# david-cortes/cmfrec

Hardware: AMD Instinct MI355X
Metric: ALS rows/sec ((users+items)/iteration time), implicit ALS-CG k=50 fp64 (higher is better)
Workload: dtype f64

## Files before the change

cmfrec_amd/_lib.py:

```python
import ctypes as C
import os

import numpy as np

_HERE = os.path.dirname(os.path.abspath(__file__))
LIBDIR = os.environ.get("CMFREC_HIP_LIBDIR") or os.path.join(_HERE, "lib")

RETURN_CODES = {0: "ok", 1: "out of memory", 2: "invalid or unsupported input", 3: "interrupted",
                4: "HIP runtime failure"}


class Model(C.Structure):
    _fields_ = [(n, C.c_int32) for n in (
        "implicit", "m", "n", "k", "k_main", "k_user", "k_item", "user_bias", "item_bias",
        "scale_lam", "scale_lam_sideinfo", "use_cg", "precondition_cg", "max_cg_steps",
        "p", "q", "m_u", "n_i")] + [("lam", C.c_double), ("w_user", C.c_double), ("w_item", C.c_double)] + \
        [(n, C.c_int32) for n in ("row_begin", "row_end", "col_begin", "col_end", "m_x", "n_x")]


class ModelF(C.Structure):
    _fields_ = [(n, C.c_int32) for n in (
        "implicit", "m", "n", "k", "k_main", "k_user", "k_item", "user_bias", "item_bias",
        "scale_lam", "scale_lam_sideinfo", "use_cg", "precondition_cg", "max_cg_steps",
        "p", "q", "m_u", "n_i")] + [("lam", C.c_float), ("w_user", C.c_float), ("w_item", C.c_float)] + \
        [(n, C.c_int32) for n in ("row_begin", "row_end", "col_begin", "col_end", "m_x", "n_x")]


EXPORTED = [
    "fit_collective_implicit_als", "fit_collective_explicit_als",
    "factors_collective_explicit_multiple", "factors_collective_implicit_multiple", "cmfrec_hip_factors_multiple", "cmfrec_hip_factors_multiple_l1",
    "cmfrec_hip_optimizeA_implicit", "cmfrec_hip_optimizeA_explicit", "cmfrec_hip_optimizeA_explicit_weighted",
    "cmfrec_hip_optimizeA_dense_full", "cmfrec_hip_optimizeA_collective", "cmfrec_hip_optimizeA_collective_sparse", "cmfrec_hip_topN_batch",
    "cmfrec_hip_ranker_create", "cmfrec_hip_ranker_topN", "cmfrec_hip_ranker_kernel_ms", "cmfrec_hip_ranker_launch_shape", "cmfrec_hip_ranker_destroy",
    "cmfrec_hip_session_create", "cmfrec_hip_session_destroy", "cmfrec_hip_last_error", "cmfrec_hip_last_error_code",
    "cmfrec_hip_session_set_X", "cmfrec_hip_session_set_A_parts", "cmfrec_hip_session_nparts", "cmfrec_hip_session_part_range", "cmfrec_hip_session_stream_wait_part", "cmfrec_hip_session_set_X_coo", "cmfrec_hip_session_set_X_coo_weighted", "cmfrec_hip_session_set_X_weighted", "cmfrec_hip_session_set_X_coo_device", "cmfrec_hip_session_precompute", "cmfrec_hip_session_init_biases", "cmfrec_hip_session_get_X", "cmfrec_hip_session_set_factors", "cmfrec_hip_session_get_factors",
    "cmfrec_hip_session_set_sideinfo", "cmfrec_hip_session_set_sideinfo_local", "cmfrec_hip_session_sideinfo_partial", "cmfrec_hip_session_sideinfo_finish", "cmfrec_hip_session_set_nonneg", "cmfrec_hip_session_set_l1", "cmfrec_hip_session_set_lam_unique", "cmfrec_hip_session_set_scale_bias_const", "cmfrec_hip_session_set_NA_as_zero_X", "cmfrec_hip_session_set_zero_rows", "cmfrec_hip_session_set_closed_form_rows", "cmfrec_hip_session_set_lambda_multipliers", "cmfrec_hip_session_set_implicit_features", "cmfrec_hip_session_get_implicit_features", "cmfrec_hip_session_set_sideinfo_sparse", "cmfrec_hip_session_update", "cmfrec_hip_session_iterate",
    "cmfrec_hip_session_sync", "cmfrec_hip_session_device_ptr", "cmfrec_hip_session_stream",
    "cmfrec_hip_session_after_gather", "cmfrec_hip_session_kernel_time",
    "cmfrec_hip_session_reset_timers", "cmfrec_hip_session_bin_overlaps", "cmfrec_hip_session_vh_mode", "cmfrec_hip_session_vh_min", "cmfrec_hip_session_lowrank_info", "cmfrec_hip_session_bin_stats", "cmfrec_hip_sizeof_real", "cmfrec_hip_sizeof_model", "cmfrec_hip_build_info", "cmfrec_hip_reload_switches", "cmfrec_hip_selftest_lanes", "cmfrec_hip_exchange_plan", "cmfrec_hip_gemm_probe", "cmfrec_hip_sym_eig", "precompute_collective_explicit", "precompute_collective_implicit", "topN_old_collective_explicit", "topN_old_collective_implicit", "cmfrec_hip_random_parallel",
]

_cache = {}


def lib_path(dtype):
    suffix = "double" if np.dtype(dtype) == np.float64 else "float"
    return os.path.join(LIBDIR, "libcmfrec_hip_%s.so" % suffix)


def load(dtype=np.float64):
    dtype = np.dtype(dtype).type
    if dtype not in (np.float64, np.float32):
        raise ValueError("dtype must be float64 or float32")
    if dtype in _cache:
        return _cache[dtype]
    path = lib_path(dtype)
    if not os.path.exists(path):
        raise ImportError(
            "%s is missing: the HIP extension has not been built (run __graft_entry__.build() or "
            "`make -C cmfrec_amd/csrc`). cmfrec_amd has no CPU fallback." % path)
    if os.environ.get("CMFREC_AMD_NO_TORCH_PRELOAD") != "1":
        try:
            import torch
        except ImportError:
            pass
    lib = C.CDLL(path)
    lib.cmfrec_hip_last_error.restype = C.c_char_p
    lib.cmfrec_hip_build_info.restype = C.c_char_p
    lib.cmfrec_hip_session_create.restype = C.c_void_p
    lib.cmfrec_hip_ranker_create.restype = C.c_void_p
    lib.cmfrec_hip_ranker_destroy.restype = None
    lib.cmfrec_hip_session_device_ptr.restype = C.c_void_p
    lib.cmfrec_hip_session_stream.restype = C.c_void_p
    assert lib.cmfrec_hip_sizeof_real() == np.dtype(dtype).itemsize
    mirror = Model if dtype is np.float64 else ModelF
    if lib.cmfrec_hip_sizeof_model() != C.sizeof(mirror):
        raise RuntimeError("cmfrec_amd: the ctypes mirror of cmfrec_hip_model (%d bytes) does not match the library (%d)"
                           % (C.sizeof(mirror), lib.cmfrec_hip_sizeof_model()))
    _cache[dtype] = lib
    return lib


def real(dtype):
    return C.c_double if np.dtype(dtype) == np.float64 else C.c_float


def ptr(a):
    return None if a is None else a.ctypes.data_as(C.c_void_p)


def check(rc, lib, what, interrupt_ok=False):
    if rc == 0 or (rc == 3 and interrupt_ok):
        return
    msg = lib.cmfrec_hip_last_error()
    msg = msg.decode() if msg else ""
    if rc == 1:
        raise MemoryError("%s: out of memory. %s" % (what, msg))
    if rc == 3:
        raise InterruptedError("%s: procedure was interrupted" % what)
    raise RuntimeError("%s failed with code %d (%s). %s" % (what, rc, RETURN_CODES.get(rc, "?"), msg))
```

cmfrec_amd/csrc/cg_kernels.hpp:

```cpp
#pragma once
#include <hip/hip_runtime.h>
#include <stdint.h>
#include <type_traits>

#include "lanes.hpp"

namespace cmfhip {

constexpr int WAVE = 64;
constexpr int TILE = 64;
constexpr int MAX_W = 8;
#ifndef CMF_CG_WAVES_PER_SIMD
#define CMF_CG_WAVES_PER_SIMD 2
#endif
#ifndef CMF_CG_WAVES_PER_SIMD_F32
#define CMF_CG_WAVES_PER_SIMD_F32 3
#endif
#ifndef CMF_CG_WAVES_PER_SIMD_LOW
#define CMF_CG_WAVES_PER_SIMD_LOW 3
#endif
constexpr int CG_NTSEL_MAX_S = 7;
template <typename T, int W, int NRES_, int NTSEL = 0> constexpr int cg_waves_per_simd()
{
    if (sizeof(T) == 8 && NTSEL == 1 && W <= 8) return CMF_CG_WAVES_PER_SIMD_LOW;
// ... 931 lines not shown
        for (int q = 0; q < 4; q++) {
            const f32x2 *g = reinterpret_cast<const f32x2 *>(G) + (jj * 4 + q) * gram_ld2(S) + ll;
#pragma unroll
            for (int s = 0; s < S; s++) v[q][s] = g[8 * s];
        }
    }
};
template <int S>
__device__ __forceinline__ void gram_pass_regs(const GramRegs<float, S> &R, float wdist, PassAcc<float> &out)
{
    float wts[8];
    wts[0] = lanes::bcast8<0>(wdist); wts[1] = lanes::bcast8<1>(wdist); wts[2] = lanes::bcast8<2>(wdist);
    wts[3] = lanes::bcast8<3>(wdist); wts[4] = lanes::bcast8<4>(wdist); wts[5] = lanes::bcast8<5>(wdist);
    wts[6] = lanes::bcast8<6>(wdist); wts[7] = lanes::bcast8<7>(wdist);
#pragma unroll
    for (int q = 0; q < 4; q++) {
        const f32x2 w2 = f32x2{wts[2 * q], wts[2 * q + 1]};
#pragma unroll
        for (int s = 0; s < S; s++) out.v[s] += w2 * R.v[q][s];
    }
}
template <typename T, int S>
__device__ __forceinline__ void gram_pass_regs(const GramRegs<T, S> &R, T wdist, PassAcc<T> &out)
{
    T wts[8];
    wts[0] = lanes::bcast8<0>(wdist); wts[1] = lanes::bcast8<1>(wdist); wts[2] = lanes::bcast8<2>(wdist);
    wts[3] = lanes::bcast8<3>(wdist); wts[4] = lanes::bcast8<4>(wdist); wts[5] = lanes::bcast8<5>(wdist);
    wts[6] = lanes::bcast8<6>(wdist); wts[7] = lanes::bcast8<7>(wdist);
#pragma unroll
    for (int t = 0; t < 8; t++)
#pragma unroll
        for (int s = 0; s < S; s++) out.v[s] += wts[t] * R.v[t][s];
}

template <bool NEG, int S>
__device__ __forceinline__ void gram_pass_regs_w(const GramRegs<float, S> &R, const float (&wts)[8], PassAcc<float> &out)
{
#pragma unroll
    for (int q = 0; q < 4; q++) {
        const f32x2 w2 = f32x2{wts[2 * q], wts[2 * q + 1]};
#pragma unroll
        for (int s = 0; s < S; s++) out.v[s] = NEG ? out.v[s] - w2 * R.v[q][s] : out.v[s] + w2 * R.v[q][s];
    }
}
template <bool NEG, typename T, int S, int GR>
__device__ __forceinline__ void gram_pass_regs_w(const GramRegs<T, S, GR> &R, const T (&wts)[8], PassAcc<T> &out)
{
#pragma unroll
    for (int t = 0; t < GR; t++)
#pragma unroll
        for (int s = 0; s < S; s++) out.v[s] = NEG ? out.v[s] - wts[t] * R.v[t][s] : out.v[s] + wts[t] * R.v[t][s];
}

template <typename T, int S, bool IMPLICIT, bool GRAMX = false, int NE = 4>
__global__ void __launch_bounds__(256, (tiny_waves_per_simd<T, IMPLICIT || GRAMX>()))
cg_rows_tiny_kernel(const CgParams<T> P)
{
    static_assert(NE == 4 || NE == 2 || NE == 0, "entries per lane group");
    constexpr bool MIX = NE == 0;
    static_assert(!MIX || CMF_TINY_WAVES_PER_SIMD >= 3, "the mixed launch lives in the dynamically scheduled loop");
    using Tile = typename TinyTile<T, S, (NE == 2) ? 2 : 4>::type;
    constexpr bool GRAM = IMPLICIT || GRAMX;
    extern __shared__ __attribute__((aligned(16))) unsigned char smem_raw[];
    T *G = reinterpret_cast<T *>(smem_raw);
    constexpr bool PV = pass_vector_in_lds<T>();
    __shared__ __attribute__((aligned(16))) T s_pv[PV ? 4 : 1][PV ? 64 : 1];
    const int tid = threadIdx.x;
    const int lane = tid & 63;
    auto short_row = [&](int nnz_) -> bool { return MIX && nnz_ <= 16; };
    auto entry_of = [&](int nnz_) -> int { return (NE == 2 || short_row(nnz_)) ? (lane >> 2) : (lane >> 1); };
    const int k = P.k;
    constexpr bool GREG = tiny_greg<T, GRAM>();
    constexpr int GR = GREG ? gram_rows<T>(S) : 8;
    if (GRAM) {
        stage_gramian<T, S, GR>(G, P.BtB, k, tid, blockDim.x);
        __syncthreads();
    }
    GramRegs<T, GREG ? S : 1, GREG ? GR : 8> greg;
    if constexpr (GREG) greg.load(G, lane);
    const int nwaves = gridDim.x * 4;
    struct Pre { int idx; T x; T a; T g; };
    auto load_desc = [&](int rix_) -> RowDesc {
        RowDesc d; d.row = 0; d.nnz = 0; d.st = 0;
        if (rix_ < P.nrows) d = P.desc[rix_];
        d.row = __builtin_amdgcn_readfirstlane(d.row);
        d.nnz = __builtin_amdgcn_readfirstlane(d.nnz);
        d.st = ((unsigned long long)(unsigned)__builtin_amdgcn_readfirstlane((int)(d.st >> 32)) << 32) |
               (unsigned)__builtin_amdgcn_readfirstlane((int)(d.st & 0xffffffffu));
        return d;
    };
    auto load_pre = [&](const RowDesc &d) -> Pre {
        Pre q; q.idx = 0; q.x = T(0); q.a = T(0); q.g = T(1);
        const int ent = entry_of(d.nnz);
        if (ent < d.nnz) {
            const size_t pos = d.st + (size_t)ent;
            q.idx = P.indices[pos];
            q.x = P.values[pos];
            q.g = entry_weight<T, IMPLICIT>(P, pos);
            if (!IMPLICIT && P.bias_sub != nullptr) q.x -= P.bias_sub[q.idx];
        }
        if (d.nnz > 0 && lane < k) q.a = P.A[(size_t)d.row * P.lda + lane];
        return q;
    };
    auto load_tile_ne = [&](Tile &t_, const T *Bm_, size_t ldb_, int k_, int idx_, int cnt_, int lane_) {
        if constexpr (NE != 2) load_tile4<T, S>(t_, Bm_, ldb_, k_, idx_, cnt_, lane_);
        else load_tile2<T, S>(t_, Bm_, ldb_, k_, idx_, cnt_, lane_);
    };
    auto solve = [&](const RowDesc &d, const Pre &pr, const Tile &tile, auto short_tag) {
        constexpr bool T2 = NE == 2 || decltype(short_tag)::value;
        const int nnz = d.nnz;
        T lam = P.lam, lam_last = P.lam_last;
        if (GRAMX && P.kc > 0) {
            if (P.scale_lam || P.scale_lam_sideinfo) {
                T mult = row_lam_mult(P, d.row, nnz);
                if (P.scale_lam_sideinfo) mult += (T)P.p_side;
                lam *= mult; lam_last *= mult;
            }
        } else if (!IMPLICIT && P.scale_lam) {
            const T mult = row_lam_mult(P, d.row, nnz);
            lam *= mult;
            if (!P.scale_bias_const) lam_last *= mult;
        }
        const bool valid = (T2 ? (lane >> 2) : (lane >> 1)) < nnz;
        T a_d = pr.a;
        auto run_pass = [&](T vdist, auto mode_tag) -> T {
            constexpr int MODE = decltype(mode_tag)::value;
            asm volatile("" ::: "memory");
            T vrep[S];
            T gw[8];
            if constexpr (PV) pass_vector_lds<T, S, GR>(vdist, vrep, gw, lane, &s_pv[tid >> 6][0]);
            else replicate<T, S>(vdist, vrep, lane);
            PassAcc<T> acc;
            if (!CMF_DBG(P, 4)) {
                if constexpr (!T2) tile_pass4<T, S, IMPLICIT, MODE, decltype(tile), true>(tile, vrep, pr.x, valid, acc, lane, pr.g);
                else tile_pass2<T, S, IMPLICIT, MODE, decltype(tile), true>(tile, vrep, pr.x, valid, acc, lane, pr.g);
            } else acc.zero();
            if constexpr (GREG) {
                if (!CMF_DBG(P, 2)) {
                    if constexpr (PV) gram_pass_regs_w<MODE == 0>(greg, gw, acc);
                    else gram_pass_regs(greg, (MODE == 0) ? -vdist : vdist, acc);
                }
            }
            else if (GRAM && !CMF_DBG(P, 2)) gram_pass<T, S, 1>(G, (MODE == 0) ? -vdist : vdist, acc, lane, 0);
            T out[8];
            acc.close(out);
            return treduce8_high<T>(out, lane);
        };
        T r_d = run_pass(a_d, std::integral_constant<int, 0>{});
        r_d -= lam * a_d;
        if (!IMPLICIT && lam != lam_last && lane == k - 1) r_d -= (lam_last - lam) * a_d;
        if (GRAMX && P.rconst != nullptr && lane < k) r_d += P.rconst[(size_t)d.row * P.ldr + lane];
        if (lane >= k) r_d = T(0);
        T p_d = r_d;
        T r_old = wave_sum(r_d * r_d);
        bool done = (r_old <= (T)1e-12);
        for (int step = 0; step < P.max_cg_steps && !done; step++) {
            T Ap_d = run_pass(p_d, std::integral_constant<int, 1>{});
            Ap_d += lam * p_d;
            if (!IMPLICIT && lam != lam_last && lane == k - 1) Ap_d += (lam_last - lam) * p_d;
            if (lane >= k) Ap_d = T(0);
            T alpha = cg_div(r_old, wave_sum(Ap_d * p_d));
            a_d += alpha * p_d;
            r_d -= alpha * Ap_d;
            T r_new = wave_sum(r_d * r_d);
            if (r_new <= (T)1e-8) done = true;
            else {
                p_d = p_d * cg_div(r_new, r_old) + r_d;
                r_old = r_new;
            }
        }
        if (lane < k) P.A[(size_t)d.row * P.lda + lane] = a_d;
    };

    int rix = blockIdx.x * 4 + (tid >> 6);
#if CMF_TINY_WAVES_PER_SIMD >= 3
    {
        const int cslot = rix % CG_NCOUNTERS;
        int *const my_counter = P.counter + cslot * CG_COUNTER_STRIDE;
        const int cbase = nwaves + cslot;
        auto issue_claim = [&]() -> int {
            int v = 0;
            if (lane == 0) v = atomicAdd(my_counter, 1);
            return v;
        };
        const int c1 = issue_claim(), c2 = issue_claim();
        int rnxt = cbase + CG_NCOUNTERS * __builtin_amdgcn_readfirstlane(c1);
        int rnn = cbase + CG_NCOUNTERS * __builtin_amdgcn_readfirstlane(c2);
        RowDesc d0 = load_desc(rix), d1 = load_desc(rnxt);
        Pre p0 = load_pre(d0);
        Tile tA;
        int pend = issue_claim();
        while (rix < P.nrows) {
            const bool shrt = short_row(d0.nnz);
            if (CMF_DBG(P, 1)) {
                dbg_fill_tile<(NE == 2) ? 2 : 4, S>(tA, (T)(p0.idx & 3) * (T)0.001);
            } else if constexpr (MIX) {
                if (shrt) load_tile2<T, S>(tA, P.B, P.ldb, k, p0.idx, d0.nnz, lane);
                else load_tile_ne(tA, P.B, P.ldb, k, p0.idx, d0.nnz, lane);
            } else load_tile_ne(tA, P.B, P.ldb, k, p0.idx, d0.nnz, lane);
            RowDesc d2 = load_desc(rnn);
            Pre p1 = load_pre(d1);
            if constexpr (MIX) {
                if (shrt) solve(d0, p0, tA, std::true_type{});
                else solve(d0, p0, tA, std::false_type{});
            } else solve(d0, p0, tA, std::false_type{});
            const int r3 = cbase + CG_NCOUNTERS * __builtin_amdgcn_readfirstlane(pend);
            d0 = d1; p0 = p1; d1 = d2;
            rix = rnxt; rnxt = rnn; rnn = r3;
            pend = issue_claim();
        }
        return;
    }
#endif
    RowDesc d0 = load_desc(rix), d1 = load_desc(rix + nwaves), d2 = load_desc(rix + 2 * nwaves);
    Pre p0 = load_pre(d0);
    Tile tA, tB;
    if (d0.nnz > 0) load_tile_ne(tA, P.B, P.ldb, k, p0.idx, d0.nnz, lane);
    Pre p1 = load_pre(d1);
    while (rix < P.nrows) {
        if (d1.nnz > 0) load_tile_ne(tB, P.B, P.ldb, k, p1.idx, d1.nnz, lane);
        RowDesc d3 = load_desc(rix + 3 * nwaves);
        Pre p2 = load_pre(d2);
        solve(d0, p0, tA, std::false_type{});
        rix += nwaves;
        if (rix >= P.nrows) break;
        if (d2.nnz > 0) load_tile_ne(tA, P.B, P.ldb, k, p2.idx, d2.nnz, lane);
        RowDesc d4 = load_desc(rix + 3 * nwaves);
        Pre p3 = load_pre(d3);
        solve(d1, p1, tB, std::false_type{});
        rix += nwaves;
        d0 = d2; p0 = p2; d1 = d3; p1 = p3; d2 = d4;
    }
}

constexpr int VH_CHUNK_TILES = 4;

struct VhWork {
    int vi;
    int row;
    int cnt;
    int chunk;
    unsigned long long st;
    unsigned long long pad_;
};

template <typename T>
struct VhState {
    T *r, *p;
    T *r_old;
    int *done;
    T *part;
    const int *chunk_row;
    const int *chunk_start;
    const int *chunk_cnt;
    const int *chunk_off;
    const int *launch;
    const VhWork *work;
    int nvh, nchunks, nlaunch;
};

template <typename T, int S, bool IMPLICIT, int MODE>
__global__ void __launch_bounds__(64 * VH_CHUNK_TILES, 3)
vh_pass_kernel(const CgParams<T> P, const VhState<T> V)
// ... 439 lines not shown
```

cmfrec_amd/csrc/device.hpp:

```cpp
#pragma once
#include <hip/hip_runtime.h>
#include <algorithm>
#include <cstdio>
#include <cstdlib>
#include <cstring>
#include <numeric>
#include <string>
#include <vector>

#include "../../include/cmfrec_hip.h"
#include "device_base.hpp"
#include "cg_kernels.hpp"
#include "chol_kernels.hpp"
#include "dense_kernels.hpp"
#include "gram_cg_kernels.hpp"
#include "topn_kernels.hpp"

namespace cmfhip {

constexpr int MAX_DEVICES = 16;
constexpr int NBINS = 6;
constexpr int BIN_VHEAVY = 0;
constexpr int BIN_HEAVY = 1;
constexpr int BIN_MED4 = 2;
constexpr int BIN_MED2 = 3;
constexpr int BIN_LIGHT = 4;
constexpr int BIN_TINY = 5;
constexpr int BIN_MIN_NNZ[NBINS] = {1025, 257, 129, 65, 33, 1};
inline int vh_min_env()
{
    const int v = switches().vh_min;
    return v > 0 ? std::min(sizeof(real_t) == 4 ? BIN_MIN_NNZ[BIN_VHEAVY] : (1 << 30), std::max(258, v)) : 0;
}

struct SparseShard {
    int nrows = 0;
    size_t nnz = 0;
    int vh_min = BIN_MIN_NNZ[BIN_VHEAVY];
    size_t opp_row_bytes_hint = 50 * sizeof(real_t);
    int bin_of(long long l) const
    {
        if (l >= vh_min) return BIN_VHEAVY;
        for (int b = 1; b < NBINS; b++)
            if (l >= BIN_MIN_NNZ[b]) return b;
        return -1;
    }
    static bool gram_pays(double vh_nnz, int n_other_, size_t opp_bytes_per_row)
    {
        (void)vh_nnz; (void)opp_bytes_per_row;
        return sizeof(real_t) == 4 || n_other_ > 0;
    }
    DevBuf<size_t> p;
    DevBuf<int> i;
    DevBuf<real_t> v;
    DevBuf<real_t> w, wsum;
// ... 354 lines not shown
    volatile unsigned int *w = poison_words;
    for (int e = threadIdx.x; e < words; e += 256) w[e] = 0xFFFFFFFFu;
}
inline void poison_lds(hipStream_t st, int num_cus)
{
    if (!switches().poison_lds) return;
    constexpr int BYTES = 80 * 1024;
    static thread_local bool attr_set = false;
    if (!attr_set) {
        HIP_CHECK(hipFuncSetAttribute((const void *)poison_lds_kernel, hipFuncAttributeMaxDynamicSharedMemorySize, BYTES));
        attr_set = true;
    }
    hipLaunchKernelGGL(poison_lds_kernel, dim3(num_cus * 4), dim3(256), BYTES, st, BYTES / 4);
    HIP_CHECK(hipGetLastError());
}

template <int S, bool IMPLICIT, int W, int RPB, bool GRAMX = false, int NRES_ = 0, int NTSEL = 0>
inline void launch_cg_bin(const DeviceInfo &dev, CgParams<real_t> P, int first, int count, BinTimers *tm, int bin, hipStream_t st, int counter_set = -1)
{
    if (count <= 0) return;
    EventPair ev{nullptr, nullptr};
    if (tm) {
        HIP_CHECK(hipEventCreate(&ev.a));
        HIP_CHECK(hipEventCreate(&ev.b));
        HIP_CHECK(hipEventRecord(ev.a, st));
    }
    poison_lds(st, dev.num_cus);
    P.order += first;
    P.desc += first;
    P.nrows = count;
    P.counter = dev.row_counter.ptr + cg_counter_offset(counter_set >= 0 ? counter_set : bin);
    constexpr int threads = 64 * W * RPB;
    size_t smem = (((IMPLICIT || GRAMX) ? (size_t)gram_elems<real_t>(S) : 0) + (size_t)RPB * 2 * W * 64) * sizeof(real_t);
    auto kern = cg_rows_kernel<real_t, S, IMPLICIT, W, RPB, GRAMX, NRES_, NTSEL>;
    static thread_local int bpc_dev[MAX_DEVICES] = {0};
    int &blocks_per_cu = bpc_dev[std::min(std::max(dev.device, 0), MAX_DEVICES - 1)];
    if (blocks_per_cu == 0) {
        if (smem > 48 * 1024)
            HIP_CHECK(hipFuncSetAttribute((const void *)kern, hipFuncAttributeMaxDynamicSharedMemorySize, (int)smem));
        int nb = 0;
        HIP_CHECK(hipOccupancyMaxActiveBlocksPerMultiprocessor(&nb, kern, threads, smem));
        blocks_per_cu = std::max(1, nb);
    }
    int teams_needed = (count + RPB - 1) / RPB;
    int grid = std::min(teams_needed, dev.num_cus * blocks_per_cu);
    hipLaunchKernelGGL(kern, dim3(grid), dim3(threads), smem, st, P);
    HIP_CHECK(hipGetLastError());
    if (tm) {
        HIP_CHECK(hipEventRecord(ev.b, st));
        tm->ev[bin].push_back(ev);
    }
}

template <int S, bool IMPLICIT, bool GRAMX = false>
inline void launch_cg_tiny(const DeviceInfo &dev, CgParams<real_t> P, int first, int count, BinTimers *tm, hipStream_t st, int n_gt16)
{
    if (count <= 0) return;
    EventPair ev{nullptr, nullptr};
    if (tm) {
        HIP_CHECK(hipEventCreate(&ev.a));
        HIP_CHECK(hipEventCreate(&ev.b));
        HIP_CHECK(hipEventRecord(ev.a, st));
    }
    poison_lds(st, dev.num_cus);
    constexpr bool tiny16_on = true;
    const int count_le16 = std::min(count, std::max(0, first + count - std::max(first, n_gt16)));
    size_t smem = ((IMPLICIT || GRAMX) ? (size_t)gram_elems<real_t>(S) : 0) * sizeof(real_t);
    const int di = std::min(std::max(dev.device, 0), MAX_DEVICES - 1);
    CgParams<real_t> P1 = P;
    P1.order += first;
    P1.desc += first;
    P1.nrows = count;
    P1.counter = dev.row_counter.ptr + cg_counter_offset(BIN_TINY);
    {
        const bool mixed = tiny16_on && count_le16 > 0;
        auto kern = mixed ? cg_rows_tiny_kernel<real_t, S, IMPLICIT, GRAMX, 0> : cg_rows_tiny_kernel<real_t, S, IMPLICIT, GRAMX, 4>;
        static thread_local int bpc_dev[MAX_DEVICES][2] = {{0}};
        int &blocks_per_cu = bpc_dev[di][mixed ? 1 : 0];
        if (blocks_per_cu == 0) {
            int nb = 0;
            HIP_CHECK(hipOccupancyMaxActiveBlocksPerMultiprocessor(&nb, kern, 256, smem));
            blocks_per_cu = std::max(1, nb);
        }
        const int grid = std::min((count + 3) / 4, dev.num_cus * blocks_per_cu);
        hipLaunchKernelGGL(kern, dim3(grid), dim3(256), smem, st, P1);
    }
    HIP_CHECK(hipGetLastError());
    if (tm) {
        HIP_CHECK(hipEventRecord(ev.b, st));
        tm->ev[BIN_TINY].push_back(ev);
    }
}

void launch_gram_wave(dim3 grid, hipStream_t st, const CgParams<real_t> &P, const GramParams<real_t> &G, bool implicit, int rem);

template <bool GRAMX>
inline bool vh_takes_gram(int k, const SparseShard &X)
{
    if (GRAMX || k > 16 * GRAM_NTT) return false;
    return (switches().vh != 0) ? switches().vh == 2 : X.prefer_gram((size_t)k * sizeof(real_t));
}

template <int S, bool IMPLICIT, bool GRAMX = false>
inline void launch_cg_vheavy(const DeviceInfo &dev_, CgParams<real_t> P, const SparseShard &X, BinTimers *tm, hipStream_t st)
{
    const int nvh = X.bin_rows[BIN_VHEAVY];
    if (nvh <= 0) return;
    struct { hipStream_t stream; int num_cus; } dev{st, dev_.num_cus};
    EventPair ev{nullptr, nullptr};
    if (tm) {
        HIP_CHECK(hipEventCreate(&ev.a));
        HIP_CHECK(hipEventCreate(&ev.b));
        HIP_CHECK(hipEventRecord(ev.a, dev.stream));
    }
    if (vh_takes_gram<GRAMX>(P.k, X)) {
        GramParams<real_t> G;
        G.sl_vrow = X.sl_vrow.ptr; G.sl_first = X.sl_first.ptr; G.sl_count = X.sl_count.ptr; G.row_sl_off = X.row_sl_off.ptr;
        G.part = X.gram_part.ptr; G.n_slices = X.n_slices; G.nvh = nvh;
        P.nrows = nvh;
#ifdef CMF_CG_DEBUG
        if (switches().debug_ticks) {
            static unsigned long long *d_t = nullptr;
            unsigned long long h[4];
            if (d_t == nullptr) { HIP_CHECK(hipMalloc((void **)&d_t, sizeof(h))); HIP_CHECK(hipMemset(d_t, 0, sizeof(h))); }
            else {
                HIP_CHECK(hipDeviceSynchronize());
                HIP_CHECK(hipMemcpy(h, d_t, sizeof(h), hipMemcpyDeviceToHost));
                if (h[1] > 0)
                    fprintf(stderr, "gram_wave: %.0f ticks per wave, %llu waves, %llu slices, %llu nnz: %.1f ticks per nnz and wave\n",
                            (double)h[0] / h[1], h[1], h[2], h[3], (double)h[0] / (double)h[3]);
                HIP_CHECK(hipMemset(d_t, 0, sizeof(h)));
            }
// ... 328 lines not shown
```

cmfrec_amd/csrc/device_base.hpp:

```cpp
#pragma once
#include <hip/hip_runtime.h>
#include <cstdio>
#include <cstdlib>
#include <cstring>
#include <functional>
#include <new>
#include <string>

#include "../../include/cmfrec_hip.h"

namespace cmfhip {

extern thread_local std::string g_last_error;
extern thread_local int g_last_rc;

struct HipError {
    int code;
};

inline void hip_check(hipError_t e, const char *what, const char *file, int line)
{
    if (e == hipSuccess) return;
    char buf[512];
    snprintf(buf, sizeof buf, "cmfrec_hip: %s failed: %s (%s:%d)", what, hipGetErrorString(e), file, line);
    g_last_error = buf;
    fprintf(stderr, "%s\n", buf);
    throw HipError{e == hipErrorOutOfMemory ? 1 : 4};
}
#define HIP_CHECK(x) ::cmfhip::hip_check((x), #x, __FILE__, __LINE__)

inline int guarded(const std::function<int()> &f)
{
    try {
        return f();
    } catch (const HipError &e) {
        return e.code;
    } catch (const std::bad_alloc &) {
        g_last_error = "cmfrec_hip: host out of memory";
        return 1;
    }
}

struct Switches {
    bool poison_lds = false;
    int vh_min = 0;
    int vh = 0;
    bool gram_slice = false;
    int bins_par = 2;
    bool nt_split = true;
    bool cg_generic = false;
    int chol = 0;
    int parts_coop = 1;
    int chol_wg = 2;
    int gramk = -1;
    int gramk_batch = 0;
    int lowrank = -1;
    bool topn_wide = false;
    int topn_tiles = 0;
    bool eig_jacobi = false;
    int debug_skip = 0;
    bool debug_ticks = false;
    void reload()
    {
        auto str = [](const char *n) -> const char * { const char *v = getenv(n); return (v != nullptr && v[0] != 0) ? v : nullptr; };
        auto num = [&](const char *n, int dflt) -> int { const char *v = str(n); return v ? atoi(v) : dflt; };
        poison_lds = str("CMFREC_HIP_POISON_LDS") != nullptr;
        vh_min = num("CMFREC_HIP_VH_MIN", 0);
        const char *v = str("CMFREC_HIP_VH");
        vh = !v ? 0 : strcmp(v, "stream") == 0 ? 1 : strcmp(v, "gram") == 0 ? 2 : 1;
        v = str("CMFREC_HIP_GRAM_KERNEL"); gram_slice = v && strcmp(v, "slice") == 0;
        bins_par = num("CMFREC_HIP_BINS_PAR", 2);
        nt_split = num("CMFREC_HIP_NT_SPLIT", 1) != 0;
        v = str("CMFREC_HIP_CG_KERNEL"); cg_generic = v && strcmp(v, "generic") == 0;
        v = str("CMFREC_HIP_CHOL"); chol = !v ? 0 : strcmp(v, "rows") == 0 ? 1 : strcmp(v, "noslices") == 0 ? 2 : 0;
        parts_coop = num("CMFREC_HIP_PARTS_COOP", 1);
        chol_wg = num("CMFREC_HIP_CHOL_WG", 2);
        if (chol_wg == 1) chol_wg = 2;
        gramk = num("CMFREC_HIP_GRAMK", -1);
        gramk_batch = num("CMFREC_HIP_GRAMK_BATCH", 0);
        lowrank = num("CMFREC_HIP_LOWRANK", -1);
        v = str("CMFREC_HIP_TOPN"); topn_wide = v && strcmp(v, "wide") == 0;
        topn_tiles = num("CMFREC_HIP_TOPN_TILES", 0);
        v = str("CMFREC_HIP_EIG"); eig_jacobi = v && strcmp(v, "jacobi") == 0;
        debug_skip = num("CMFREC_HIP_CG_SKIP", num("CMFREC_HIP_CHOL_SKIP", num("CMFREC_HIP_WAVE_SKIP", 0)));
        debug_ticks = str("CMFREC_HIP_GRAM_TICKS") != nullptr || str("CMFREC_HIP_CHOL_TICKS") != nullptr;
    }
};
inline Switches &switches_mut() { static Switches sw; static bool first = (sw.reload(), true); (void)first; return sw; }
inline const Switches &switches() { return switches_mut(); }

template <typename T>
struct DevBuf {
    T *ptr = nullptr;
    size_t n = 0;
    bool owned = true;
    DevBuf() = default;
    DevBuf(const DevBuf &) = delete;
    DevBuf &operator=(const DevBuf &) = delete;
    ~DevBuf() { release(); }
    void release()
    {
        if (ptr && owned) (void)hipFree(ptr);
        ptr = nullptr;
        n = 0;
    }
    void alloc(size_t count)
    {
        release();
        n = count;
        owned = true;
        if (count) HIP_CHECK(hipMalloc((void **)&ptr, count * sizeof(T)));
        if (count && switches().poison_lds) {
            HIP_CHECK(hipMemset(ptr, 0xFF, count * sizeof(T)));
            HIP_CHECK(hipDeviceSynchronize());
        }
    }
    void alloc_at_least(size_t count)
    {
        if (n < count) alloc(count);
    }
    void upload(const T *host, size_t count, hipStream_t st)
    {
        if (count > n) alloc(count);
        if (count) HIP_CHECK(hipMemcpyAsync(ptr, host, count * sizeof(T), hipMemcpyDefault, st));
    }
// ... 10 lines not shown
```

cmfrec_amd/csrc/session.hip:

```cpp
#include "device.hpp"
#include "coo_device.hpp"
#include "chol_wave_kernels.hpp"
#include "gramk_kernels.hpp"
#include "lowrank_kernels.hpp"
#include "eig_kernels.hpp"
#include "gram_cg_wide_kernels.hpp"
#include <dlfcn.h>
#include <functional>
#include <memory>
#include <new>

namespace cmfhip {

thread_local std::string g_last_error;
thread_local int g_last_rc = 0;

CgVariant cg_variant_from_env() { return switches().cg_generic ? CgVariant::Generic : CgVariant::Auto; }

inline dim3 grid1d(size_t n, int block = 256) { return dim3((unsigned)((n + block - 1) / block)); }
hipError_t launch_chol_wg8(int num_cus, bool border, int waves_per_row, hipStream_t st, const CholParams<real_t> &W, const RowDesc *desc, const CholSlices<real_t> &SL);
hipError_t launch_chol_parts_coop(int num_cus, bool border, int depth, hipStream_t st, const CholParams<real_t> &W, const RowDesc *desc, const CholSlices<real_t> &SL);

struct CholCall {
    real_t *A; size_t lda;
// ... 3438 lines not shown
        init_device(dev, -1);
        DevBuf<real_t> dA, dQ, dQt, dL;
        DevBuf<double> W, V, D, E, Tau;
        DevBuf<int> info;
        const size_t nn = (size_t)n * n;
        dA.upload(A, nn, dev.stream); dQ.alloc(nn); dQt.alloc(nn); dL.alloc((size_t)n);
        W.alloc(nn); V.alloc(nn); D.alloc((size_t)n); E.alloc((size_t)n); Tau.alloc((size_t)n); info.alloc(1);
        HIP_CHECK(hipMemsetAsync(info.ptr, 0, sizeof(int), dev.stream));
        hipEvent_t e0, e1;
        HIP_CHECK(hipEventCreate(&e0)); HIP_CHECK(hipEventCreate(&e1));
        const bool wide = n > 288;
        const int rows = wide ? 32 : 64;
        const size_t smem = ((size_t)n * rows + 4 * (size_t)n) * sizeof(double);
        auto kern = wide ? eig_ql_rows_kernel<real_t, 32> : eig_ql_rows_kernel<real_t, 64>;
        HIP_CHECK(hipFuncSetAttribute((const void *)kern, hipFuncAttributeMaxDynamicSharedMemorySize, 160 * 1024));
        for (int r = 0; r < std::max(reps, 1) + 1; r++) {
            if (r == 1) HIP_CHECK(hipEventRecord(e0, dev.stream));
            if (method == 0 || method == 2) {
                hipLaunchKernelGGL(eig_tridiag_kernel<real_t>, dim3(1), dim3(EIG_TRIDIAG_THREADS), 0, dev.stream, dA.ptr, n, W.ptr, D.ptr, E.ptr, Tau.ptr);
                if (method == 0 || r == 0)
                    hipLaunchKernelGGL(kern, dim3((n + rows - 1) / rows), dim3(64), smem, dev.stream, n, W.ptr, D.ptr, E.ptr, Tau.ptr, dQ.ptr, dQt.ptr,
                                       (size_t)n, dL.ptr, info.ptr);
            } else
                hipLaunchKernelGGL(jacobi_eig_kernel<real_t>, dim3(1), dim3(1024), 0, dev.stream, dA.ptr, n, W.ptr, V.ptr, dQ.ptr, dQt.ptr, (size_t)n,
                                   dL.ptr, 30, sizeof(real_t) == 4 ? 1e-9 : 1e-13);
            HIP_CHECK(hipGetLastError());
        }
        HIP_CHECK(hipEventRecord(e1, dev.stream));
        HIP_CHECK(hipEventSynchronize(e1));
        float t = 0;
        HIP_CHECK(hipEventElapsedTime(&t, e0, e1));
        if (ms) *ms = (double)t / std::max(reps, 1);
        int h_info = 0;
        HIP_CHECK(hipMemcpyAsync(&h_info, info.ptr, sizeof(int), hipMemcpyDeviceToHost, dev.stream));
        dQ.download(Q, nn, dev.stream); dL.download(lam, (size_t)n, dev.stream);
        HIP_CHECK(hipStreamSynchronize(dev.stream));
        (void)hipEventDestroy(e0); (void)hipEventDestroy(e1);
        if (h_info != 0) { g_last_error = "cmfrec_hip_sym_eig: a QL iteration did not converge"; return 4; }
        return 0;
    });
}

#ifdef CMF_CG_TICKS
extern "C" int cmfrec_hip_debug_cg_ticks(unsigned long long *out)
{
    unsigned long long *buf = cg_ticks_buffer();
    HIP_CHECK(hipDeviceSynchronize());
    HIP_CHECK(hipMemcpy(out, buf, 32 * sizeof(unsigned long long), hipMemcpyDeviceToHost));
    HIP_CHECK(hipMemset(buf, 0, 32 * sizeof(unsigned long long)));
    return 0;
}
#endif

extern "C" int cmfrec_hip_selftest_lanes(void)
{
    int bad = -1;
    int rc = guarded([&]() {
        DeviceInfo dev;
        init_device(dev, -1);
        DevBuf<real_t> d;
        d.alloc(17 * 64);
        hipLaunchKernelGGL(lanes_selftest_kernel, dim3(1), dim3(64), 0, dev.stream, d.ptr);
        HIP_CHECK(hipGetLastError());
        std::vector<real_t> h(17 * 64);
        d.download(h.data(), h.size(), dev.stream);
        HIP_CHECK(hipStreamSynchronize(dev.stream));
        auto X = [](int l) { return (double)(l * 3 + 1); };
        auto Y = [](int l) { return (double)(1000 + l); };
        bad = 0;
        for (int l = 0; l < 64; l++) {
            double e[17];
            e[0] = X(l ^ 1); e[1] = X(l ^ 2); e[2] = X(l ^ 4); e[3] = X(l ^ 8);
            e[4] = (l & 4) ? Y(l ^ 4) : X(l ^ 4);
            e[5] = (l & 8) ? Y(l ^ 8) : X(l ^ 8);
            e[6] = (l < 32) ? X(l) + X(l + 32) : Y(l - 32) + Y(l);
            e[7] = (l & 16) ? Y(l - 16) + Y(l) : X(l) + X(l + 16);
            e[8] = X((l & ~7) | 0); e[9] = X((l & ~7) | 3); e[10] = X((l & ~7) | 5); e[11] = X((l & ~7) | 7);
            double s = 0; for (int j = 0; j < 64; j++) s += X(j);
            e[12] = s;
            { int b = l & 7; double t = 0; for (int j = 0; j < 8; j++) t += (double)(((l & ~7) | j) + 100 * b); e[13] = t; }
            { int b = l >> 3; double t = 0; for (int j = 0; j < 8; j++) t += (double)(((l & 7) | (j << 3)) + 100 * b); e[14] = t; }
            e[15] = X(l ^ 7);
            e[16] = (double)(((l & ~7) | 6) * 5 + 2);
            for (int c = 0; c < 17; c++)
                if ((double)h[c * 64 + l] != e[c]) {
                    if (bad < 8) fprintf(stderr, "lanes selftest: case %d lane %d got %g expected %g\n", c, l, (double)h[c * 64 + l], e[c]);
                    bad++;
                }
        }
        return 0;
    });
    return rc ? -rc : bad;
}
```

include/cmfrec_hip.h:

```cpp
#ifndef CMFREC_HIP_H
#define CMFREC_HIP_H
#include <stddef.h>
#include <stdint.h>
#include <stdbool.h>

#ifdef CMFREC_HIP_FLOAT
typedef float real_t;
#else
typedef double real_t;
#endif
typedef int int_t;

#ifdef __cplusplus
extern "C" {
#endif


int_t fit_collective_implicit_als(
    real_t *A, real_t *B,
    real_t *C, real_t *D,
    bool reset_values, int_t seed,
    real_t *U_colmeans, real_t *I_colmeans,
    int_t m, int_t n, int_t k,
    int_t ixA[], int_t ixB[], real_t *X, size_t nnz,
// ... 291 lines not shown
    real_t *biasB, real_t glob_mean, bool NA_as_zero_X,
    real_t *U_colmeans, bool NA_as_zero_U,
    int_t k, int_t k_user, int_t k_item, int_t k_main,
    bool user_bias,
    bool nonneg,
    real_t lam, real_t *lam_unique,
    bool scale_lam, bool scale_lam_sideinfo,
    bool scale_bias_const, real_t scaling_biasA,
    real_t w_main, real_t w_user, real_t w_implicit,
    real_t *B_plus_bias,
    real_t *BtB,
    real_t *TransBtBinvBt,
    real_t *BtXbias,
    real_t *BeTBeChol,
    real_t *BiTBi,
    real_t *TransCtCinvCt,
    real_t *CtCw,
    real_t *CtUbias);
int_t precompute_collective_implicit(
    real_t *B, int_t n,
    real_t *C, int_t p,
    real_t *U_colmeans, bool NA_as_zero_U,
    int_t k, int_t k_user, int_t k_item, int_t k_main,
    real_t lam, real_t w_main, real_t w_user, real_t w_main_multiplier,
    bool nonneg,
    bool extra_precision,
    real_t *BtB,
    real_t *BeTBe,
    real_t *BeTBeChol,
    real_t *CtUbias);

int_t topN_old_collective_explicit(
    real_t *a_vec, real_t a_bias,
    real_t *A, real_t *biasA, int_t row_index,
    real_t *B,
    real_t *biasB,
    real_t glob_mean,
    int_t k, int_t k_user, int_t k_item, int_t k_main,
    int_t *include_ix, int_t n_include,
    int_t *exclude_ix, int_t n_exclude,
    int_t *outp_ix, real_t *outp_score,
    int_t n_top, int_t n, int_t n_max, bool include_all_X, int nthreads);
int_t topN_old_collective_implicit(
    real_t *a_vec,
    real_t *A, int_t row_index,
    real_t *B,
    int_t k, int_t k_user, int_t k_item, int_t k_main,
    int_t *include_ix, int_t n_include,
    int_t *exclude_ix, int_t n_exclude,
    int_t *outp_ix, real_t *outp_score,
    int_t n_top, int_t n, int nthreads);

int cmfrec_hip_selftest_lanes(void);
int cmfrec_hip_gemm_probe(int M, int N, int K, int transa, int reps, double *ms_own, double *ms_rocblas, double *max_rel_diff);
int cmfrec_hip_sym_eig(int n, const real_t *A, real_t *Q, real_t *lam, int method, int reps, double *ms);

int cmfrec_hip_random_parallel(real_t *A, size_t sizeA, real_t *B, size_t sizeB, int_t seed, bool normal);

int cmfrec_hip_exchange_plan(int D, const int *bb, int *out, int cap);

int cmfrec_hip_sizeof_real(void);
int cmfrec_hip_sizeof_model(void);
const char *cmfrec_hip_build_info(void);
void cmfrec_hip_reload_switches(void);

#ifdef __cplusplus
}
#endif
#endif
```

Measured before the change: 166.7 million.

## Prefetch tiny-bin CG row images into LDS via async global_load_lds

Adds a prefetching variant of the tiny-row CG kernel. While the current row is being solved, the B rows for the next row's nonzeros are gathered straight into per-wave LDS images with global_load_lds. The variant is enabled by default when the Gramian lives in registers and alignment allows, and it deepens the row-claim pipeline to three rows ahead. The goal is to hide gather latency behind the solve, at the cost of more LDS per block (possibly lower occupancy) and more complex wait handling. It also adds a launch counter and optional tick instrumentation.

Result: slower. 165.0 million (-1.1%).

```diff
diff --git a/cmfrec_amd/_lib.py b/cmfrec_amd/_lib.py
--- a/cmfrec_amd/_lib.py
+++ b/cmfrec_amd/_lib.py
@@ -30,6 +30,7 @@
     "fit_collective_implicit_als", "fit_collective_explicit_als",
     "factors_collective_explicit_multiple", "factors_collective_implicit_multiple", "cmfrec_hip_factors_multiple", "cmfrec_hip_factors_multiple_l1",
     "cmfrec_hip_optimizeA_implicit", "cmfrec_hip_optimizeA_explicit", "cmfrec_hip_optimizeA_explicit_weighted",
+    "cmfrec_hip_tiny_prefetch_launches",
     "cmfrec_hip_optimizeA_dense_full", "cmfrec_hip_optimizeA_collective", "cmfrec_hip_optimizeA_collective_sparse", "cmfrec_hip_topN_batch",
     "cmfrec_hip_ranker_create", "cmfrec_hip_ranker_topN", "cmfrec_hip_ranker_kernel_ms", "cmfrec_hip_ranker_launch_shape", "cmfrec_hip_ranker_destroy",
     "cmfrec_hip_session_create", "cmfrec_hip_session_destroy", "cmfrec_hip_last_error", "cmfrec_hip_last_error_code",
@@ -67,6 +68,7 @@
     lib = C.CDLL(path)
     lib.cmfrec_hip_last_error.restype = C.c_char_p
     lib.cmfrec_hip_build_info.restype = C.c_char_p
+    lib.cmfrec_hip_tiny_prefetch_launches.restype = C.c_longlong
     lib.cmfrec_hip_session_create.restype = C.c_void_p
     lib.cmfrec_hip_ranker_create.restype = C.c_void_p
     lib.cmfrec_hip_ranker_destroy.restype = None
diff --git a/cmfrec_amd/csrc/cg_kernels.hpp b/cmfrec_amd/csrc/cg_kernels.hpp
--- a/cmfrec_amd/csrc/cg_kernels.hpp
+++ b/cmfrec_amd/csrc/cg_kernels.hpp
@@ -1007,7 +1007,8 @@
         for (int s = 0; s < S; s++) out.v[s] = NEG ? out.v[s] - wts[t] * R.v[t][s] : out.v[s] + wts[t] * R.v[t][s];
 }
 
-template <typename T, int S, bool IMPLICIT, bool GRAMX = false, int NE = 4>
+template <typename T> constexpr int tiny_image_bytes(int S) { return 32 * 8 * S * (int)sizeof(T); }
+template <typename T, int S, bool IMPLICIT, bool GRAMX = false, int NE = 4, bool PF = false>
 __global__ void __launch_bounds__(256, (tiny_waves_per_simd<T, IMPLICIT || GRAMX>()))
 cg_rows_tiny_kernel(const CgParams<T> P)
 {
@@ -1035,21 +1036,28 @@
     if constexpr (GREG) greg.load(G, lane);
     const int nwaves = gridDim.x * 4;
     struct Pre { int idx; T x; T a; T g; };
-    auto load_desc = [&](int rix_) -> RowDesc {
+    auto load_desc_raw = [&](int rix_) -> RowDesc {
         RowDesc d; d.row = 0; d.nnz = 0; d.st = 0;
         if (rix_ < P.nrows) d = P.desc[rix_];
+        return d;
+    };
+    auto uniform_desc = [&](RowDesc d) -> RowDesc {
         d.row = __builtin_amdgcn_readfirstlane(d.row);
         d.nnz = __builtin_amdgcn_readfirstlane(d.nnz);
         d.st = ((unsigned long long)(unsigned)__builtin_amdgcn_readfirstlane((int)(d.st >> 32)) << 32) |
                (unsigned)__builtin_amdgcn_readfirstlane((int)(d.st & 0xffffffffu));
         return d;
     };
-    auto load_pre = [&](const RowDesc &d) -> Pre {
-        Pre q; q.idx = 0; q.x = T(0); q.a = T(0); q.g = T(1);
+    auto load_desc = [&](int rix_) -> RowDesc { return uniform_desc(load_desc_raw(rix_)); };
+    auto load_pre_idx = [&](const RowDesc &d) -> int {
+        const int ent = entry_of(d.nnz);
+        return (ent < d.nnz) ? P.indices[d.st + (size_t)ent] : 0;
+    };
+    auto load_pre_rest = [&](const RowDesc &d, int idx_) -> Pre {
+        Pre q; q.idx = idx_; q.x = T(0); q.a = T(0); q.g = T(1);
         const int ent = entry_of(d.nnz);
         if (ent < d.nnz) {
             const size_t pos = d.st + (size_t)ent;
-            q.idx = P.indices[pos];
             q.x = P.values[pos];
             q.g = entry_weight<T, IMPLICIT>(P, pos);
             if (!IMPLICIT && P.bias_sub != nullptr) q.x -= P.bias_sub[q.idx];
@@ -1057,6 +1065,7 @@
         if (d.nnz > 0 && lane < k) q.a = P.A[(size_t)d.row * P.lda + lane];
         return q;
     };
+    auto load_pre = [&](const RowDesc &d) -> Pre { return load_pre_rest(d, load_pre_idx(d)); };
     auto load_tile_ne = [&](Tile &t_, const T *Bm_, size_t ldb_, int k_, int idx_, int cnt_, int lane_) {
         if constexpr (NE != 2) load_tile4<T, S>(t_, Bm_, ldb_, k_, idx_, cnt_, lane_);
         else load_tile2<T, S>(t_, Bm_, ldb_, k_, idx_, cnt_, lane_);
@@ -1138,6 +1147,103 @@
             if (lane == 0) v = atomicAdd(my_counter, 1);
             return v;
         };
+#ifdef CMF_CG_TICKS
+        unsigned long long tk_wait = 0, tk_pass = 0, tk_rows = 0;
+        const unsigned long long tk_begin = CMF_TICK();
+#endif
+        if constexpr (PF) {
+            static_assert(GREG && NE != 2, "the row images take the LDS of a Gramian that lives in registers");
+            __syncthreads();
+            const unsigned rowb = (unsigned)k * (unsigned)sizeof(T);
+            const int ppr = (int)(rowb >> 4);
+            const int epi = __builtin_amdgcn_readfirstlane(64 / ppr);
+            const int el = lane / ppr;
+            const bool fill_lane = el < epi;
+            const unsigned ldb_bytes = (unsigned)(P.ldb * sizeof(T));
+            const char *const src0 = reinterpret_cast<const char *>(P.B) + 16 * (lane - el * ppr);
+            unsigned char *const img = smem_raw + (tid >> 6) * tiny_image_bytes<T>(S);
+            auto fill = [&](int my_idx, int nnz_) {
+                const int nfill = max(nnz_, 1);
+                const int sh = short_row(nnz_) ? 4 : 3;
+                constexpr int U = 8;
+                for (int e0 = 0; e0 < nfill; e0 += U * epi) {
+                    unsigned it[U];
+#pragma unroll
+                    for (int u = 0; u < U; u++) it[u] = (unsigned)__builtin_amdgcn_ds_bpermute((e0 + u * epi + el) << sh, my_idx);
+#pragma unroll
+                    for (int u = 0; u < U; u++) {
+                        const int eu = e0 + u * epi;
+                        if (eu < nfill) {
+                            if (fill_lane && eu + el < nfill)
+                                __builtin_amdgcn_global_load_lds((const __attribute__((address_space(1))) void *)(src0 + (unsigned long long)it[u] * ldb_bytes),
+                                                                 (__attribute__((address_space(3))) void *)(img + (unsigned)eu * rowb), 16, 0, 0);
+                        }
+                    }
+                }
+            };
+            auto read_tile = [&](Tile &tile, int cnt, auto nt_tag) {
+                constexpr int NT = decltype(nt_tag)::value;
+                const int jj = lane >> 3, ll = lane & 7;
+                const int col_last = min(ll + 8 * (S - 1), k - 1) - ll;
+#pragma unroll
+                for (int t = 0; t < NT; t++) {
+                    const int e = ((jj * NT + t) < cnt) ? (jj * NT + t) : 0;
+                    const T *rp = reinterpret_cast<const T *>(img + (unsigned)e * rowb) + ll;
+#pragma unroll
+                    for (int s = 0; s < S; s++) tile.set(t, s, rp[(s < S - 1) ? 8 * s : col_last]);
+                }
+            };
+            const int c1 = issue_claim(), c2 = issue_claim(), c3 = issue_claim();
+            int r1 = cbase + CG_NCOUNTERS * __builtin_amdgcn_readfirstlane(c1);
+            int r2 = cbase + CG_NCOUNTERS * __builtin_amdgcn_readfirstlane(c2);
+            int r3 = cbase + CG_NCOUNTERS * __builtin_amdgcn_readfirstlane(c3);
+            RowDesc d0 = load_desc(rix), d1 = load_desc(r1);
+            Pre p0 = load_pre(d0);
+            int i1 = load_pre_idx(d1);
+            RowDesc d2raw = load_desc_raw(r2);
+            int pend = issue_claim();
+            Tile tA;
+            if (rix < P.nrows && !CMF_DBG(P, 1)) fill(p0.idx, d0.nnz);
+            while (rix < P.nrows) {
+#ifdef CMF_CG_TICKS
+                const unsigned long long tk0 = CMF_TICK();
+#endif
+                asm volatile("s_waitcnt vmcnt(0)" ::: "memory");
+#ifdef CMF_CG_TICKS
+                const unsigned long long tk1 = CMF_TICK();
+                tk_wait += tk1 - tk0;
+#endif
+                const RowDesc d2 = uniform_desc(d2raw);
+                const int r4 = cbase + CG_NCOUNTERS * __builtin_amdgcn_readfirstlane(pend);
+                asm volatile("" : "+v"(p0.x), "+v"(p0.a), "+v"(p0.g), "+v"(i1));
+                const bool shrt = short_row(d0.nnz);
+                if (CMF_DBG(P, 1)) dbg_fill_tile<4, S>(tA, (T)(p0.idx & 3) * (T)0.001);
+                else if constexpr (MIX) {
+                    if (shrt) read_tile(tA, d0.nnz, std::integral_constant<int, 2>{});
+                    else read_tile(tA, d0.nnz, std::integral_constant<int, 4>{});
+                } else read_tile(tA, d0.nnz, std::integral_constant<int, 4>{});
+                asm volatile("s_waitcnt lgkmcnt(0)" ::: "memory");
+                if (r1 < P.nrows && !CMF_DBG(P, 1)) fill(i1, d1.nnz);
+                asm volatile("" ::: "memory");
+                RowDesc d3raw = load_desc_raw(r3);
+                const int i2 = load_pre_idx(d2);
+                Pre p1 = load_pre_rest(d1, i1);
+                pend = issue_claim();
+                if constexpr (MIX) {
+                    if (shrt) solve(d0, p0, tA, std::true_type{});
+                    else solve(d0, p0, tA, std::false_type{});
+                } else solve(d0, p0, tA, std::false_type{});
+#ifdef CMF_CG_TICKS
+                tk_pass += CMF_TICK() - tk1; tk_rows += 1;
+#endif
+                d0 = d1; d1 = d2; d2raw = d3raw; p0 = p1; i1 = i2;
+                rix = r1; r1 = r2; r2 = r3; r3 = r4;
+            }
+#ifdef CMF_CG_TICKS
+            cg_ticks_flush(P.ticks, 4, tk_wait, tk_pass, tk_rows, CMF_TICK() - tk_begin, lane);
+#endif
+            return;
+        }
         const int c1 = issue_claim(), c2 = issue_claim();
         int rnxt = cbase + CG_NCOUNTERS * __builtin_amdgcn_readfirstlane(c1);
         int rnn = cbase + CG_NCOUNTERS * __builtin_amdgcn_readfirstlane(c2);
@@ -1155,15 +1261,27 @@
             } else load_tile_ne(tA, P.B, P.ldb, k, p0.idx, d0.nnz, lane);
             RowDesc d2 = load_desc(rnn);
             Pre p1 = load_pre(d1);
+#ifdef CMF_CG_TICKS
+            const unsigned long long tk0 = CMF_TICK();
+            asm volatile("s_waitcnt vmcnt(0)" ::: "memory");
+            const unsigned long long tk1 = CMF_TICK();
+            tk_wait += tk1 - tk0;
+#endif
             if constexpr (MIX) {
                 if (shrt) solve(d0, p0, tA, std::true_type{});
                 else solve(d0, p0, tA, std::false_type{});
             } else solve(d0, p0, tA, std::false_type{});
+#ifdef CMF_CG_TICKS
+            tk_pass += CMF_TICK() - tk1; tk_rows += 1;
+#endif
             const int r3 = cbase + CG_NCOUNTERS * __builtin_amdgcn_readfirstlane(pend);
             d0 = d1; p0 = p1; d1 = d2;
             rix = rnxt; rnxt = rnn; rnn = r3;
             pend = issue_claim();
         }
+#ifdef CMF_CG_TICKS
+        cg_ticks_flush(P.ticks, 4, tk_wait, tk_pass, tk_rows, CMF_TICK() - tk_begin, lane);
+#endif
         return;
     }
 #endif
diff --git a/cmfrec_amd/csrc/device.hpp b/cmfrec_amd/csrc/device.hpp
--- a/cmfrec_amd/csrc/device.hpp
+++ b/cmfrec_amd/csrc/device.hpp
@@ -1,6 +1,7 @@
 #pragma once
 #include <hip/hip_runtime.h>
 #include <algorithm>
+#include <atomic>
 #include <cstdio>
 #include <cstdlib>
 #include <cstring>
@@ -461,6 +462,8 @@
     }
 }
 
+inline std::atomic<long long> g_tiny_prefetch_launches{0};
+
 template <int S, bool IMPLICIT, bool GRAMX = false>
 inline void launch_cg_tiny(const DeviceInfo &dev, CgParams<real_t> P, int first, int count, BinTimers *tm, hipStream_t st, int n_gt16)
 {
@@ -481,12 +484,25 @@
     P1.desc += first;
     P1.nrows = count;
     P1.counter = dev.row_counter.ptr + cg_counter_offset(BIN_TINY);
+    constexpr bool PF_BUILD = tiny_greg<real_t, IMPLICIT || GRAMX>();
+    const bool prefetch = PF_BUILD && switches().tiny_prefetch && ((uintptr_t)P.B % 16) == 0 && (P.ldb * sizeof(real_t)) % 16 == 0 &&
+                          ((size_t)P.k * sizeof(real_t)) % 16 == 0;
+    if (prefetch) {
+        smem = std::max(smem, (size_t)4 * tiny_image_bytes<real_t>(S));
+        g_tiny_prefetch_launches.fetch_add(1, std::memory_order_relaxed);
+    }
     {
         const bool mixed = tiny16_on && count_le16 > 0;
-        auto kern = mixed ? cg_rows_tiny_kernel<real_t, S, IMPLICIT, GRAMX, 0> : cg_rows_tiny_kernel<real_t, S, IMPLICIT, GRAMX, 4>;
-        static thread_local int bpc_dev[MAX_DEVICES][2] = {{0}};
-        int &blocks_per_cu = bpc_dev[di][mixed ? 1 : 0];
+        using Kern = void (*)(const CgParams<real_t>);
+        Kern kern = mixed ? cg_rows_tiny_kernel<real_t, S, IMPLICIT, GRAMX, 0> : cg_rows_tiny_kernel<real_t, S, IMPLICIT, GRAMX, 4>;
+        if constexpr (PF_BUILD) {
+            if (prefetch) kern = mixed ? cg_rows_tiny_kernel<real_t, S, IMPLICIT, GRAMX, 0, true> : cg_rows_tiny_kernel<real_t, S, IMPLICIT, GRAMX, 4, true>;
+        }
+        static thread_local int bpc_dev[MAX_DEVICES][2][2] = {{{0}}};
+        int &blocks_per_cu = bpc_dev[di][mixed ? 1 : 0][prefetch ? 1 : 0];
         if (blocks_per_cu == 0) {
+            if (smem > 48 * 1024)
+                HIP_CHECK(hipFuncSetAttribute((const void *)kern, hipFuncAttributeMaxDynamicSharedMemorySize, (int)smem));
             int nb = 0;
             HIP_CHECK(hipOccupancyMaxActiveBlocksPerMultiprocessor(&nb, kern, 256, smem));
             blocks_per_cu = std::max(1, nb);
diff --git a/cmfrec_amd/csrc/device_base.hpp b/cmfrec_amd/csrc/device_base.hpp
--- a/cmfrec_amd/csrc/device_base.hpp
+++ b/cmfrec_amd/csrc/device_base.hpp
@@ -48,6 +48,7 @@
     bool gram_slice = false;
     int bins_par = 2;
     bool nt_split = true;
+    bool tiny_prefetch = true;
     bool cg_generic = false;
     int chol = 0;
     int parts_coop = 1;
@@ -71,6 +72,7 @@
         v = str("CMFREC_HIP_GRAM_KERNEL"); gram_slice = v && strcmp(v, "slice") == 0;
         bins_par = num("CMFREC_HIP_BINS_PAR", 2);
         nt_split = num("CMFREC_HIP_NT_SPLIT", 1) != 0;
+        tiny_prefetch = num("CMFREC_HIP_TINY_PREFETCH", 1) != 0;
         v = str("CMFREC_HIP_CG_KERNEL"); cg_generic = v && strcmp(v, "generic") == 0;
         v = str("CMFREC_HIP_CHOL"); chol = !v ? 0 : strcmp(v, "rows") == 0 ? 1 : strcmp(v, "noslices") == 0 ? 2 : 0;
         parts_coop = num("CMFREC_HIP_PARTS_COOP", 1);
diff --git a/cmfrec_amd/csrc/session.hip b/cmfrec_amd/csrc/session.hip
--- a/cmfrec_amd/csrc/session.hip
+++ b/cmfrec_amd/csrc/session.hip
@@ -3514,6 +3514,8 @@
 }
 #endif
 
+extern "C" long long cmfrec_hip_tiny_prefetch_launches(void) { return g_tiny_prefetch_launches.load(std::memory_order_relaxed); }
+
 extern "C" int cmfrec_hip_selftest_lanes(void)
 {
     int bad = -1;
diff --git a/include/cmfrec_hip.h b/include/cmfrec_hip.h
--- a/include/cmfrec_hip.h
+++ b/include/cmfrec_hip.h
@@ -367,6 +367,7 @@
     int_t n_top, int_t n, int nthreads);
 
 int cmfrec_hip_selftest_lanes(void);
+long long cmfrec_hip_tiny_prefetch_launches(void);
 int cmfrec_hip_gemm_probe(int M, int N, int K, int transa, int reps, double *ms_own, double *ms_rocblas, double *max_rel_diff);
 int cmfrec_hip_sym_eig(int n, const real_t *A, real_t *Q, real_t *lam, int method, int reps, double *ms);
 
```
